# Zeng-Yan/centermask2

Measured on AMD Instinct MI355X. Metric: images/sec whole-node (V2-39-eSE 3x800x1280), higher is better.
Workload: dtype f32; 1 GPU; Full CenterMask2 V-39-eSE (VoVNetV2-FPN + FCOS + CenterROIHeads/SAG-Mask/MaskIoU + ROIAlignV2), bs=8 per GPU, 3x800x1280, end-to-end (BASELINE configs[3]); global_batch=8, per_gpu_batch=8, parallelism=dp1, launch=hip-graph, collective=none, weights=seeded random-init, reference state-dict keys

## Files before the change

### centermask2_amd/csrc/conv.hip

```cpp
#include <algorithm>

#include "conv_args.hpp"

namespace cmk {

__global__ __launch_bounds__(256) void splitk_reduce_kernel(const float* __restrict__ ws, int ksplit, long total_pix, int cout_pad,
                                                           const float* __restrict__ scale, const float* __restrict__ shift, int Cout,
                                                           int relu_upto, const float* __restrict__ res, int res_cs, int res_co,
                                                           float* __restrict__ y, int y_cs, int y_co) {
    const int c4n = cout_pad >> 2;
    const long total = total_pix * c4n;
    for (long i = (long)blockIdx.x * 256 + threadIdx.x; i < total; i += (long)gridDim.x * 256) {
        const long pix = i / c4n;
        const int co = (int)(i - pix * c4n) * 4;
        if (co >= Cout) continue;
        f32x4 s = {0.f, 0.f, 0.f, 0.f};
        for (int z = 0; z < ksplit; ++z) {
            const f32x4 v = *reinterpret_cast<const f32x4*>(ws + ((long)z * total_pix + pix) * cout_pad + co);
            s.x += v.x; s.y += v.y; s.z += v.z; s.w += v.w;
        }
#pragma unroll
        for (int j = 0; j < 4; ++j) {
            const int c = co + j;
            if (c < Cout) {
                float v = s[j] * scale[c] + shift[c];
                if (res) v += res[pix * res_cs + res_co + c];
                if (c < relu_upto) v = fmaxf(v, 0.f);
                y[pix * y_cs + y_co + c] = v;
            }
        }
    }
}

static int validate(const cmk_conv_desc* d) {
    if (!d || !d->x || !d->w || !d->y || !d->scale || !d->shift) return fail(CMK_EINVAL, "conv: null pointer%s", "");
    if (d->ksize != 1 && d->ksize != 3) return fail(CMK_EINVAL, "conv: ksize must be 1 or 3%s", "");
    if (d->stride != 1 && d->stride != 2) return fail(CMK_EINVAL, "conv: stride must be 1 or 2%s", "");
    if (d->ksize == 1 && d->stride != 1) return fail(CMK_EINVAL, "conv: 1x1 stride 2 unsupported%s", "");
    if (d->Cin <= 0 || (d->Cin & 15)) return fail(CMK_EINVAL, "conv: Cin (%s%ld) must be a positive multiple of 16", "", d->Cin);
    if (d->Cout <= 0 || d->N <= 0 || d->H <= 0 || d->W <= 0) return fail(CMK_EINVAL, "conv: empty shape%s", "");
    if ((d->x_cs & 3) || (d->x_co & 3)) return fail(CMK_EINVAL, "conv: input view must be 16-byte aligned per pixel%s", "");
    if (((uintptr_t)d->x & 15) || ((uintptr_t)d->w & 15)) return fail(CMK_EINVAL, "conv: x/w must be 16-byte aligned%s", "");
    if (d->x_co + d->Cin > d->x_cs || d->y_co + d->Cout > d->y_cs) return fail(CMK_EINVAL, "conv: channel view out of range%s", "");
    if (d->res_mode < 0 || d->res_mode > 2 || (d->res_mode && !d->res)) return fail(CMK_EINVAL, "conv: bad residual%s", "");
    if ((d->in_scale == nullptr) != (d->in_shift == nullptr)) return fail(CMK_EINVAL, "conv: in_scale and in_shift come together%s", "");
    if (d->in_scale && d->ksize == 1 && ((long)d->H * d->W) % 256) return fail(CMK_EINVAL, "conv: input affine on a 1x1 conv needs H*W %% 256 == 0%s", "");
    if (d->pool_ws && d->ksize != 1) return fail(CMK_EINVAL, "conv: pooled sums are for 1x1 convs%s", "");
    return CMK_OK;
}

static int validate_multi(const cmk_conv_desc* descs, int n) {
    if (!descs || n < 1 || n > MAXP) return fail(CMK_EINVAL, "conv_multi: need 1..%s%ld problems", "", MAXP);
    bool same_w = true;
    for (int i = 0; i < n; ++i) {
        int rc = validate(&descs[i]);
        if (rc) return rc;
        const cmk_conv_desc *a = &descs[0], *b = &descs[i];
        same_w = same_w && b->w == a->w && b->w_wino == a->w_wino && b->w_wino6 == a->w_wino6 && b->w_split == a->w_split && b->w_splith == a->w_splith;
        if (b->Cin != a->Cin || b->Cout != a->Cout || b->ksize != a->ksize || b->stride != a->stride ||
            b->relu_upto != a->relu_upto || b->in_relu != a->in_relu || b->x_cs != a->x_cs || b->x_co != a->x_co || b->y_cs != a->y_cs ||
            b->y_co != a->y_co || b->res_mode != 0 || b->tune_wm != a->tune_wm || b->tune_sc != a->tune_sc || b->tune_wn != a->tune_wn || (b->in_scale == nullptr) != (a->in_scale == nullptr) ||
            b->gn_ws != a->gn_ws || b->gn_groups != a->gn_groups || b->splitk > 1 || b->pool_ws)
            return fail(CMK_EINVAL, "conv_multi: problems must share channels/views/flags and carry no residual%s", "");
    }
    if ((!same_w || n > 5) && (descs[0].tune_wm != 6 || descs[0].tune_wn != 1) && descs[0].tune_wm != 11)
        return fail(CMK_EINVAL, "conv_multi: different weights per problem / more than 5 problems need tune_wm 6, tune_wn 1 (the F(4x4) map kernels)%s", "");
    for (int i = 0; i < n; ++i)
        if (descs[0].tune_wm == 6 && !descs[i].w_wino6) return fail(CMK_EINVAL, "conv_multi: w_wino6 missing%s", "");
    return CMK_OK;
}

static void fill_problem(ConvProblem& p, const cmk_conv_desc* d) {
    p.x = d->x; p.y = d->y; p.scale = d->scale; p.shift = d->shift;
    p.in_scale = d->in_scale; p.in_shift = d->in_shift;
    p.w = d->w_wino6;
    p.N = d->N; p.H = d->H; p.W = d->W;
    p.Ho = out_size(d->H, d->stride);
    p.Wo = out_size(d->W, d->stride);
    p.tiles_h = p.tiles_w = p.tile_begin = 0;
    p.total_pix = (long)p.N * p.Ho * p.Wo;
}

static int setup_gn(ConvArgs& a, const cmk_conv_desc* d) {
    const int cpg = d->gn_groups > 0 ? d->Cout / d->gn_groups : 0;
    if (d->relu_upto != 0 || d->gn_groups < 1 || d->Cout % d->gn_groups || cpg > 32 || (cpg & (cpg - 1)))
        return fail(CMK_EINVAL, "conv: fused GroupNorm statistics need relu_upto == 0 and a power-of-two group width <= 32%s", "");
    a.gn_ws = d->gn_ws; a.gn_cpg = cpg; a.gn_groups = d->gn_groups;
    return CMK_OK;
}

static int pointwise_mt(const cmk_conv_desc* d, int n) {
    const int cout32 = (d->Cout + 31) / 32;
    const long total_pix = (long)d->N * d->H * d->W;
    if (d->ksize != 1 || n != 1 || cout32 <= 7 || (d->Cin & 31) || d->in_scale || d->in_relu || d->gn_ws || total_pix * d->x_cs * 4 >= (1L << 31))
        return 0;
    if (d->splitk > 1 && (d->tune_wm != 8 || !d->splitk_ws || d->res_mode == 2 || d->pool_ws || (d->Cin >> 4) % (2 * d->splitk))) return 0;
    if (d->res_mode == 2 && ((d->W & 1) || d->pool_ws || (long)d->N * d->Hr * d->Wr * d->res_cs * 4 >= (1L << 31))) return 0;
    if (d->tune_wm == 8) return (d->tune_wn == 4 || d->tune_wn == 2) ? d->tune_wn : 0;
    if (d->tune_wm == 10) return (d->w_split && d->tune_wn == 4 && d->res_mode != 1 && d->splitk <= 1) ? 4 : 0;
    if (d->tune_wm == 12) return (d->w_splith && d->tune_wn == 4 && d->res_mode != 1 && d->splitk <= 1) ? 4 : 0;
    if (d->tune_wm || d->tune_sc || d->tune_wn) return 0;
    const long ctiles = cdiv(cout32, 4);
    const long wg2 = ((total_pix + 127) / 128) * ctiles, wg4 = ((total_pix + 255) / 256) * ctiles;
    return wg2 >= 256 ? (wg4 >= 1024 ? 4 : 2) : 0;
}

static int gather_mt(const cmk_conv_desc* d, int n) {
    const int cout32 = (d->Cout + 31) / 32;
    const long in_pix = (long)d->N * d->H * d->W;
    const long out_pix = (long)d->N * (d->stride == 1 ? d->H : (d->H - 1) / 2 + 1) * (d->stride == 1 ? d->W : (d->W - 1) / 2 + 1);
    if (d->ksize != 3 || n != 1 || (cout32 != 4 && cout32 <= 7) || (d->Cin & 31) || d->in_scale || d->in_relu || d->res_mode == 2 ||
        d->gn_ws || d->pool_ws || in_pix * d->x_cs * 4 >= (1L << 31) || d->H >= 32768 || d->W >= 32768)
        return 0;
    if (d->splitk > 1 && (d->tune_wm != 9 || !d->splitk_ws || (9 * (d->Cin >> 4)) % (2 * d->splitk))) return 0;
    if (d->tune_wm == 9) return (d->tune_wn == 4 || d->tune_wn == 2) ? d->tune_wn : 0;
// ... 105 lines not shown
        if (d->tune_wn != 1 && d->tune_wn != 2) return fail(CMK_EINVAL, "conv: tune_wm 6 takes tune_wn 1 (12x40 map tiles) or 2 (pairs of RoI maps up to 16x14)%s", "");
        if (d->tune_sc == 64) return launch_wino6s(a, d->tune_wn == 2 ? 1 : 0, st, plan);
        return launch_wino6(a, d->tune_wn == 2 ? 1 : 0, pair, st, plan);
    }
    a.ksplit = d->splitk > 1 ? d->splitk : 1;
    a.ws = d->splitk_ws;
    if (d->pool_ws && !pointwise_mt(d, n)) return fail(CMK_EINVAL, "conv: pooled sums are produced by the pointwise GEMM kernel only (cmk_conv_pool_rows)%s", "");
    a.pool_ws = d->pool_ws;
    if (d->tune_wm == 8) {
        if (d->ksize != 1 || cout32 <= 7) return fail(CMK_EINVAL, "conv: pointwise variant needs a 1x1 conv with Cout > 224%s", "");
        a.cout_pad = cout_pad128;
        if (a.ksplit > 1 && !pointwise_mt(d, n)) return fail(CMK_EINVAL, "conv: pointwise variant: split-K not available for this conv%s", "");
        return launch_pw(a, d->tune_wn, st, plan);
    }
    if (d->tune_wm == 10 || d->tune_wm == 12) {
        const bool f16 = d->tune_wm == 12;
        if (!(d->ksize == 1 ? pointwise_mt(d, n) : gather_mt(d, n)) || (f16 && !(d->w_splith_scale > 0.f)))
            return fail(CMK_EINVAL, f16 ? "conv: the fp16-split variant needs w_splith, w_splith_scale and a conv the pointwise GEMM kernel takes (1x1, or 3x3 in its gather form)%s"
                                        : "conv: the bf16-split variant needs w_split and a conv the pointwise GEMM kernel takes (1x1, or 3x3 in its gather form)%s", "");
        a.cout_pad = cout_pad128;
        a.w = reinterpret_cast<const float*>(f16 ? d->w_splith : d->w_split);
        if (f16) a.p[0].acc_scale = d->w_splith_scale;
        a.ksplit = 1;
        a.ga_stride = d->ksize == 3 ? d->stride : 0;
        return launch_pw_split(a, f16 ? 2 : 1, st, plan);
    }
    if (d->tune_wm == 11) {
        if (d->ksize != 3 || d->stride != 1 || !d->w_splith || d->splitk > 1 || d->res_mode != 0 || d->in_relu || d->pool_ws)
            return fail(CMK_EINVAL, "conv: the direct fp16-split variant needs w_splith and a plain 3x3 stride-1 conv%s", "");
        for (int i = 0; i < n; ++i) {
            if (!descs[i].w_splith || !(descs[i].w_splith_scale > 0.f)) return fail(CMK_EINVAL, "conv: w_splith / w_splith_scale missing%s", "");
            a.p[i].w = reinterpret_cast<const float*>(descs[i].w_splith);
            a.p[i].acc_scale = descs[i].w_splith_scale;
        }
        a.cout_pad = cout_pad128;
        a.ksplit = 1;
        return launch_sp3(a, d->tune_wn, d->tune_sc, st, plan);
    }
    if (d->tune_wm == 9) {
        const int mt = gather_mt(d, n);
        if (!mt) return fail(CMK_EINVAL, "conv: pointwise gather variant not available for this conv%s", "");
        a.cout_pad = cout_pad128;
        a.ga_stride = d->stride;
        return launch_pw(a, mt, st, plan);
    }
    if (d->tune_wm == 7) {
        if (d->ksize != 3 || n != 1 || d->res_mode == 2 || d->in_scale || (d->tune_wn != 1 && d->tune_wn != 2 && d->tune_wn != 4))
            return fail(CMK_EINVAL, "conv: gather variant not available for this conv%s", "");
        const int cout_pad32 = cout32 <= 7 ? cout32 : cdiv(cout32, 4) * 4;
        if (cout_pad32 % d->tune_wn) return fail(CMK_EINVAL, "conv: gather variant: Cout tiles %% WN != 0%s", "");
        a.cout_pad = cout_pad32 * 32;
        a.ga_stride = d->stride;
        return launch_igemm_gather(a, d->tune_wn, cout_pad32 / d->tune_wn, st, plan);
    }
    const Variant v{d->tune_wm, d->tune_sc, d->tune_wn};
    if (!variant_ok(d->ksize * d->ksize, d->stride, cout32, v.wm, v.sc, v.wn)) return fail(CMK_EINVAL, "conv: variant not available for this shape%s", "");
    return launch_igemm(a, d->ksize, d->stride, cout32, v, st, plan);
}

static int run(const cmk_conv_desc* descs, int n, void* stream, LaunchPlan* plan = nullptr) {
    const cmk_conv_desc* d = &descs[0];
    ConvArgs a;
    memset(&a, 0, sizeof(a));
    a.nprob = n;
    for (int i = 0; i < n; ++i) fill_problem(a.p[i], &descs[i]);
    a.w = d->w; a.res = d->res;
    a.Cin = d->Cin; a.Cout = d->Cout;
    a.x_cs = d->x_cs; a.x_co = d->x_co; a.y_cs = d->y_cs; a.y_co = d->y_co;
    a.res_cs = d->res_cs; a.res_co = d->res_co; a.res_mode = d->res_mode; a.Hr = d->Hr; a.Wr = d->Wr;
    if (a.res_mode == 2 && (a.Hr * 2 < a.p[0].Ho || a.Wr * 2 < a.p[0].Wo)) return fail(CMK_EINVAL, "conv: upsampled residual too small%s", "");
    a.relu_upto = d->relu_upto; a.in_relu = d->in_relu;
    const bool ask_gn = plan && !d->gn_ws && d->gn_groups > 0;
    const Variant v = resolve(descs, n, d->gn_ws != nullptr || ask_gn);
    cmk_conv_desc dv = *d;
    dv.tune_wm = v.wm; dv.tune_sc = v.sc; dv.tune_wn = v.wn;
    static double no_ws;
    if (ask_gn && writes_gn_records(v.wm)) dv.gn_ws = &no_ws;
    hipStream_t st = (hipStream_t)stream;
    int rc = dispatch(a, &dv, descs, n, st, plan);
    if (rc || plan) return rc;
    if (a.ksplit <= 1 && a.tail_ksplit > 1 && a.tail_tiles > 0) {
        const ConvProblem& p = a.p[0];
        const long pix0 = (long)2 * (a.total_tiles - a.tail_tiles) * p.Ho * p.Wo, tpix = p.total_pix - pix0;
        hipLaunchKernelGGL(splitk_reduce_kernel, dim3((unsigned)std::min<long>((tpix * (a.cout_pad >> 2) + 255) / 256, 256L * 32)), dim3(256), 0, st, a.ws, a.tail_ksplit,
                           tpix, a.cout_pad, p.scale, p.shift, a.Cout, a.relu_upto, (const float*)nullptr, 0, 0, p.y + pix0 * a.y_cs, a.y_cs, a.y_co);
        return check_launch("splitk_reduce (tail)");
    }
    if (a.ksplit <= 1) return rc;
    const ConvProblem& p = a.p[0];
    hipLaunchKernelGGL(splitk_reduce_kernel, dim3((unsigned)std::min<long>((p.total_pix * (a.cout_pad >> 2) + 255) / 256, 256L * 32)), dim3(256), 0, st, a.ws, a.ksplit, p.total_pix,
                       a.cout_pad, p.scale, p.shift, a.Cout, a.relu_upto, a.res_mode == 1 ? a.res : nullptr, a.res_cs, a.res_co, p.y, a.y_cs,
                       a.y_co);
    return check_launch("splitk_reduce");
}

}

extern "C" int cmk_conv_cout_pad(int Cout) {
    int c32 = (Cout + 31) / 32;
    return c32 <= 7 ? c32 * 32 : ((c32 + 3) / 4) * 128;
}

extern "C" int64_t cmk_conv_packed_floats(int Cout, int Cin, int ksize) {
    int64_t taps = (int64_t)ksize * ksize;
    int64_t nch = (Cin + 15) / 16;
    return taps * nch * cmk_conv_cout_pad(Cout) * 16;
}

extern "C" int cmk_conv_gn_tiles(int H, int W) { return ((H + 7) / 8) * ((W + 15) / 16); }

extern "C" int cmk_conv_gn_records(int H, int W, int tune_wm) {
    return tune_wm == 6 ? cmk::wino6_gn_records(H, W) : cmk::wino4r_gn_records(H, W);
}

extern "C" int64_t cmk_splith_packed_halves(int Cout, int Cin) {
    return (int64_t)((Cin + 15) / 16) * (((Cout + 127) / 128) * 4) * 2 * 64 * 8;
}

extern "C" int64_t cmk_split_packed_halves(int Cout, int Cin) {
    return (int64_t)((Cin + 15) / 16) * (((Cout + 127) / 128) * 4) * 3 * 64 * 8;
}

extern "C" int64_t cmk_wino_packed_floats(int Cout, int Cin) {
    return (int64_t)((Cin + 15) / 16) * ((Cout + 63) / 64) * 16 * 64 * 16;
}

extern "C" int cmk_conv_pool_rows(const cmk_conv_desc* d) {
    if (!d) return 0;
    const int mt = cmk::pointwise_mt(d, 1);
    return (mt && (long)d->H * d->W >= 32 * mt) ? 32 * mt : 0;
}

extern "C" int64_t cmk_conv_tail_ws_floats(const cmk_conv_desc* d) {
    if (!d) return 0;
    int tiles = 0, ways = 0;
    cmk::wino6_tail_of(d, tiles, ways);
    if (tiles <= 0 || ways <= 1) return 0;
    const int st = (d->N + 1) / 2;
    const int64_t images = d->N - 2 * (int64_t)(st - tiles);
    return (int64_t)ways * images * d->H * d->W * cmk_conv_cout_pad(d->Cout);
}

extern "C" int cmk_conv2d_nhwc(const cmk_conv_desc* d, void* stream) {
    int rc = cmk::validate(d);
    if (rc) return rc;
    return cmk::run(d, 1, stream);
}

extern "C" int cmk_conv2d_nhwc_multi(const cmk_conv_desc* descs, int n, void* stream) {
    int rc = cmk::validate_multi(descs, n);
    if (rc) return rc;
    return cmk::run(descs, n, stream);
}

extern "C" int cmk_conv_plan(const cmk_conv_desc* descs, int n, char* kernel, int kernel_cap, double* executed_flops, int* gn_records) {
    int rc = n == 1 ? cmk::validate(descs) : cmk::validate_multi(descs, n);
    if (rc) return rc;
    cmk::LaunchPlan plan;
    memset(&plan, 0, sizeof(plan));
    rc = cmk::run(descs, n, nullptr, &plan);
    if (rc) return rc;
    if (kernel && kernel_cap > 0) snprintf(kernel, kernel_cap, "%s", plan.kernel);
    if (executed_flops) *executed_flops = (double)plan.executed_flops;
    for (int i = 0; gn_records && i < n; ++i) gn_records[i] = plan.gn_records[i];
    return CMK_OK;
}

extern "C" int cmk_conv_resolve(const cmk_conv_desc* descs, int n, int with_gn_stats, int variant[3]) {
    int rc = n == 1 ? cmk::validate(descs) : cmk::validate_multi(descs, n);
    if (rc) return rc;
    if (!variant) return cmk::fail(CMK_EINVAL, "conv_resolve: null variant%s", "");
    const cmk::Variant v = cmk::resolve(descs, n, with_gn_stats || descs[0].gn_ws);
    variant[0] = v.wm; variant[1] = v.sc; variant[2] = v.wn;
// ... 3 lines not shown
```

### centermask2_amd/csrc/elementwise.hip

```cpp
#include "cmk_common.hpp"

namespace cmk {

typedef float f32x4 __attribute__((ext_vector_type(4)));
typedef float f32x16 __attribute__((ext_vector_type(16)));

__device__ __forceinline__ float nanmax(float m, float v) { return (v > m || v != v) ? v : m; }
__device__ __forceinline__ float hsigmoid3(float v) {
    v = v < 0.f ? 0.f : v;
    v = v > 6.f ? 6.f : v;
    return v / 6.0f;
}

template <int NB>
__global__ __launch_bounds__(256) void stem_conv_kernel(const float* __restrict__ x, const float* __restrict__ w,
                                                       const float* __restrict__ scale, const float* __restrict__ shift,
                                                       float* __restrict__ y, int N, int H, int W, int Ho, int Wo, long tiles) {
    const int lane = threadIdx.x & 63, wave = threadIdx.x >> 6;
    const int li = lane & 31, hh = lane >> 5;
    constexpr int Cout = NB * 32;
    float b[14][NB], sc[NB], sh[NB];
    int dlt[14], khs[14], kws[14];
#pragma unroll
    for (int s = 0; s < 14; ++s) {
// ... 74 lines not shown

__global__ __launch_bounds__(256) void subsample2_kernel(const float* __restrict__ x, int x_cs, int x_co, float* __restrict__ y, int y_cs, int y_co,
                                                        int N, int H, int W, int Ho, int Wo, int C4) {
    long total = (long)N * Ho * Wo * C4;
    for (long i = (long)blockIdx.x * 256 + threadIdx.x; i < total; i += (long)gridDim.x * 256) {
        int c4 = (int)(i % C4);
        long p = i / C4;
        int ow = (int)(p % Wo);
        int oh = (int)((p / Wo) % Ho);
        int n = (int)(p / ((long)Wo * Ho));
        *reinterpret_cast<f32x4*>(y + p * y_cs + y_co + c4 * 4) =
            *reinterpret_cast<const f32x4*>(x + (((long)n * H + 2 * oh) * W + 2 * ow) * x_cs + x_co + c4 * 4);
    }
}

__global__ __launch_bounds__(256) void ese_partial_kernel(const float* __restrict__ x, int x_cs, int x_co, float* __restrict__ ws,
                                                         int HW, int C, int chunks) {
    extern __shared__ float red[];
    const int n = blockIdx.y, chunk = blockIdx.x;
    const int G = C >> 2;
    const int ppl = G >= 256 ? 1 : 256 / G;
    const int per = cdiv(HW, chunks);
    const int p0 = chunk * per, p1 = min(HW, p0 + per);
    const float* xn = x + (long)n * HW * x_cs + x_co;
    for (int gi = threadIdx.x; gi < G * ppl; gi += 256) {
        int g = gi % G, pl = gi / G;
        f32x4 s = {0.f, 0.f, 0.f, 0.f};
        for (int p = p0 + pl; p < p1; p += ppl) {
            f32x4 v = *reinterpret_cast<const f32x4*>(xn + (long)p * x_cs + g * 4);
            s.x += v.x; s.y += v.y; s.z += v.z; s.w += v.w;
        }
        *reinterpret_cast<f32x4*>(red + pl * C + g * 4) = s;
    }
    __syncthreads();
    for (int c = threadIdx.x; c < C; c += 256) {
        float s = 0.f;
        for (int pl = 0; pl < ppl; ++pl) s += red[pl * C + c];
        ws[((long)n * chunks + chunk) * C + c] = s;
    }
}

__global__ __launch_bounds__(256) void ese_fc_kernel(const float* __restrict__ ws, const float* __restrict__ fc_w,
                                                    const float* __restrict__ fc_b, float* __restrict__ gate, int HW, int C,
                                                    int chunks) {
    extern __shared__ double smd[];
    const int n = blockIdx.y;
    const int G = C >> 2;
    const int parts = G >= 256 ? 1 : 256 / G;
    const float* wsn = ws + (long)n * chunks * C;
    for (int gi = threadIdx.x; gi < G * parts; gi += 256) {
        const int g = gi % G, part = gi / G;
        double s0 = 0.0, s1 = 0.0, s2 = 0.0, s3 = 0.0;
#pragma unroll 8
        for (int k = part; k < chunks; k += parts) {
            const f32x4 v = *reinterpret_cast<const f32x4*>(wsn + (long)k * C + g * 4);
            s0 += (double)v.x; s1 += (double)v.y; s2 += (double)v.z; s3 += (double)v.w;
        }
        double* o = smd + part * C + g * 4;
        o[0] = s0; o[1] = s1; o[2] = s2; o[3] = s3;
    }
    __syncthreads();
    for (int c = threadIdx.x; c < C; c += 256) {
        double s = 0.0;
        for (int part = 0; part < parts; ++part) s += smd[part * C + c];
        smd[c] = s / (double)HW;
    }
    __syncthreads();
    const int lane = threadIdx.x & 63, wave = threadIdx.x >> 6;
    for (int o = blockIdx.x * 16 + wave; o < min(C, (int)(blockIdx.x + 1) * 16); o += 4) {
        const float* wr = fc_w + (long)o * C;
        double s = 0.0;
        for (int c = lane * 4; c < C; c += 256) {
            f32x4 wv = *reinterpret_cast<const f32x4*>(wr + c);
            s += (double)wv.x * smd[c] + (double)wv.y * smd[c + 1] + (double)wv.z * smd[c + 2] + (double)wv.w * smd[c + 3];
        }
        s = wave_sum(s);
        if (lane == 0) {
            float v = (float)(s + (double)fc_b[o] + 3.0);
            gate[(long)n * C + o] = hsigmoid3(v);
        }
    }
}

__global__ __launch_bounds__(256) void ese_fc_pooled_kernel(const float* __restrict__ rec, int rows, const float* __restrict__ fc_w,
                                                           const float* __restrict__ fc_b, float* __restrict__ gate, int HW, int C) {
    extern __shared__ double smd[];
    const int n = blockIdx.y;
    const int G = C >> 2;
    const int parts = G >= 256 ? 1 : 256 / G;
    const long p0 = (long)n * HW;
    const long g0 = p0 / rows, g1 = (p0 + HW - 1) / rows;
    const long first = (g0 * rows == p0) ? 2 * g0 : 2 * g0 + 1;
    for (int gi = threadIdx.x; gi < G * parts; gi += 256) {
        const int g = gi % G, part = gi / G;
        double s0 = 0.0, s1 = 0.0, s2 = 0.0, s3 = 0.0;
        if (part == 0) {
            const f32x4 v = *reinterpret_cast<const f32x4*>(rec + first * C + g * 4);
            s0 = v.x; s1 = v.y; s2 = v.z; s3 = v.w;
        }
#pragma unroll 8
        for (long k = g0 + 1 + part; k <= g1; k += parts) {
            const f32x4 v = *reinterpret_cast<const f32x4*>(rec + 2 * k * C + g * 4);
            s0 += (double)v.x; s1 += (double)v.y; s2 += (double)v.z; s3 += (double)v.w;
        }
        double* o = smd + part * C + g * 4;
        o[0] = s0; o[1] = s1; o[2] = s2; o[3] = s3;
    }
    __syncthreads();
    for (int c = threadIdx.x; c < C; c += 256) {
        double s = 0.0;
        for (int part = 0; part < parts; ++part) s += smd[part * C + c];
        smd[c] = s / (double)HW;
    }
    __syncthreads();
    const int lane = threadIdx.x & 63, wave = threadIdx.x >> 6;
    for (int o = blockIdx.x * 16 + wave; o < min(C, (int)(blockIdx.x + 1) * 16); o += 4) {
        const float* wr = fc_w + (long)o * C;
        double s = 0.0;
        for (int c = lane * 4; c < C; c += 256) {
            f32x4 wv = *reinterpret_cast<const f32x4*>(wr + c);
            s += (double)wv.x * smd[c] + (double)wv.y * smd[c + 1] + (double)wv.z * smd[c + 2] + (double)wv.w * smd[c + 3];
        }
        s = wave_sum(s);
        if (lane == 0) {
            float v = (float)(s + (double)fc_b[o] + 3.0);
            gate[(long)n * C + o] = hsigmoid3(v);
        }
    }
}

__global__ __launch_bounds__(256) void ese_scale_kernel(const float* __restrict__ x, int x_cs, int x_co, const float* __restrict__ gate,
                                                       const float* __restrict__ idn, int id_cs, int id_co, float* __restrict__ y,
                                                       int y_cs, int y_co, int N, int HW, int C4) {
    long total = (long)N * HW * C4;
    for (long i = (long)blockIdx.x * 256 + threadIdx.x; i < total; i += (long)gridDim.x * 256) {
        int c4 = (int)(i % C4);
        long p = i / C4;
        int n = (int)(p / HW);
        f32x4 v = *reinterpret_cast<const f32x4*>(x + p * x_cs + x_co + c4 * 4);
        f32x4 g = *reinterpret_cast<const f32x4*>(gate + (long)n * C4 * 4 + c4 * 4);
        f32x4 o = {v.x * g.x, v.y * g.y, v.z * g.z, v.w * g.w};
        if (idn) {
            f32x4 d = *reinterpret_cast<const f32x4*>(idn + p * id_cs + id_co + c4 * 4);
            o.x += d.x; o.y += d.y; o.z += d.z; o.w += d.w;
        }
        *reinterpret_cast<f32x4*>(y + p * y_cs + y_co + c4 * 4) = o;
    }
}

__global__ __launch_bounds__(256) void upsample2x_add_kernel(float* __restrict__ y, const float* __restrict__ c, int N, int H, int W, int Hc, int Wc, int C4) {
    long total = (long)N * H * W * C4;
    for (long i = (long)blockIdx.x * 256 + threadIdx.x; i < total; i += (long)gridDim.x * 256) {
        int c4 = (int)(i % C4);
        long p = i / C4;
        int w = (int)(p % W);
        int h = (int)((p / W) % H);
        int n = (int)(p / ((long)W * H));
        const f32x4 a = *reinterpret_cast<const f32x4*>(y + i * 4);
        const f32x4 b = *reinterpret_cast<const f32x4*>(c + ((((long)n * Hc + (h >> 1)) * Wc + (w >> 1)) * C4 + c4) * 4);
        *reinterpret_cast<f32x4*>(y + i * 4) = f32x4{a.x + b.x, a.y + b.y, a.z + b.z, a.w + b.w};
    }
}

}

using namespace cmk;

extern "C" int cmk_stem_conv_nchw3(const float* x, const float* w, const float* scale, const float* shift, float* y, int N, int H,
                                   int W, int Cout, void* stream) {
    if (!x || !w || !scale || !shift || !y) return fail(CMK_EINVAL, "stem: null pointer%s", "");
    if (Cout != 32 && Cout != 64 && Cout != 128) return fail(CMK_EINVAL, "stem: Cout (%s%ld) must be 32, 64 or 128", "", (long)Cout);
    int Ho = (H - 1) / 2 + 1, Wo = (W - 1) / 2 + 1;
    long total = (long)N * Ho * Wo;
    if ((long)3 * H * W >= (1L << 31)) return fail(CMK_EINVAL, "stem: image too large%s", "");
    long tiles = (total + 31) / 32;
    unsigned grid = (unsigned)std::min<long>((tiles + 3) / 4, 256 * 16);
    if (Cout == 32)
        hipLaunchKernelGGL(stem_conv_kernel<1>, dim3(grid), dim3(256), 0, (hipStream_t)stream, x, w, scale, shift, y, N, H, W, Ho, Wo, tiles);
    else if (Cout == 64)
        hipLaunchKernelGGL(stem_conv_kernel<2>, dim3(grid), dim3(256), 0, (hipStream_t)stream, x, w, scale, shift, y, N, H, W, Ho, Wo, tiles);
    else
        hipLaunchKernelGGL(stem_conv_kernel<4>, dim3(grid), dim3(256), 0, (hipStream_t)stream, x, w, scale, shift, y, N, H, W, Ho, Wo, tiles);
    return check_launch("stem_conv");
}

extern "C" int cmk_maxpool3x3s2_ceil_nhwc(const float* x, int x_cs, int x_co, float* y, int y_cs, int y_co, int N, int H, int W, int C,
                                          const float* gate, void* stream) {
    if (!x || !y) return fail(CMK_EINVAL, "maxpool: null pointer%s", "");
    if ((C & 3) || (x_cs & 3) || (x_co & 3) || (y_cs & 3) || (y_co & 3)) return fail(CMK_EINVAL, "maxpool: channels must be multiples of 4%s", "");
    if (H < 3 || W < 3) return fail(CMK_EINVAL, "maxpool: input smaller than the window%s", "");
    int Ho = (H - 3 + 1) / 2 + 1, Wo = (W - 3 + 1) / 2 + 1;
    if ((Ho - 1) * 2 >= H) --Ho;
    if ((Wo - 1) * 2 >= W) --Wo;
    long total = (long)N * Ho * Wo * (C >> 2);
    hipLaunchKernelGGL(maxpool3_kernel, dim3(stream_grid(total)), dim3(256), 0, (hipStream_t)stream, x, x_cs, x_co, y, y_cs, y_co, N, H, W,
                       Ho, Wo, C >> 2, gate);
    return check_launch("maxpool3");
}

extern "C" int cmk_maxpool1x1s2_nhwc(const float* x, int x_cs, int x_co, float* y, int y_cs, int y_co, int N, int H, int W, int C, void* stream) {
    if (!x || !y) return fail(CMK_EINVAL, "maxpool1x1s2: null pointer%s", "");
    if ((C & 3) || (x_cs & 3) || (x_co & 3) || (y_cs & 3) || (y_co & 3) || N < 1 || H < 1 || W < 1)
        return fail(CMK_EINVAL, "maxpool1x1s2: channels must be multiples of 4, N, H, W >= 1%s", "");
    const int Ho = (H - 1) / 2 + 1, Wo = (W - 1) / 2 + 1;
    long total = (long)N * Ho * Wo * (C >> 2);
    hipLaunchKernelGGL(subsample2_kernel, dim3(stream_grid(total)), dim3(256), 0, (hipStream_t)stream, x, x_cs, x_co, y, y_cs, y_co, N, H, W, Ho, Wo,
                       C >> 2);
    return check_launch("maxpool1x1s2");
}

extern "C" int cmk_ese_gate(const float* x, int x_cs, int x_co, const float* fc_w, const float* fc_b, float* gate, float* ws,
                            int ws_chunks, int N, int HW, int C, void* stream) {
    if (!x || !fc_w || !fc_b || !gate || !ws) return fail(CMK_EINVAL, "ese_gate: null pointer%s", "");
    if ((C & 3) || (x_cs & 3) || (x_co & 3) || ws_chunks < 1) return fail(CMK_EINVAL, "ese_gate: bad shape%s", "");
    if (N < 1 || HW < 1 || C < 4) return fail(CMK_EINVAL, "ese_gate: N, H*W >= 1 and C >= 4%s", "");
    int G = C >> 2;
    int ppl = G >= 256 ? 1 : 256 / G;
    size_t lds1 = (size_t)ppl * C * sizeof(float);
    hipLaunchKernelGGL(ese_partial_kernel, dim3(ws_chunks, N), dim3(256), lds1, (hipStream_t)stream, x, x_cs, x_co, ws, HW, C, ws_chunks);
    int rc = check_launch("ese_partial");
    if (rc) return rc;
    hipLaunchKernelGGL(ese_fc_kernel, dim3(cdiv(C, 16), N), dim3(256), 2 * lds1 , (hipStream_t)stream, ws, fc_w, fc_b,
                       gate, HW, C, ws_chunks);
    return check_launch("ese_fc");
}

extern "C" int cmk_ese_gate_pooled(const float* pool_ws, int rows, const float* fc_w, const float* fc_b, float* gate, int N, int HW, int C, void* stream) {
    if (!pool_ws || !fc_w || !fc_b || !gate) return fail(CMK_EINVAL, "ese_gate_pooled: null pointer%s", "");
    if ((C & 3) || C < 4 || rows < 1 || HW < rows || N < 1) return fail(CMK_EINVAL, "ese_gate_pooled: bad shape (C %% 4, H*W >= rows)%s", "");
    const int G = C >> 2;
    const int parts = G >= 256 ? 1 : 256 / G;
    hipLaunchKernelGGL(ese_fc_pooled_kernel, dim3(cdiv(C, 16), N), dim3(256), (size_t)parts * C * sizeof(double), (hipStream_t)stream, pool_ws, rows,
                       fc_w, fc_b, gate, HW, C);
    return check_launch("ese_fc_pooled");
}

extern "C" int cmk_ese_scale(const float* x, int x_cs, int x_co, const float* gate, const float* identity, int id_cs, int id_co, float* y,
                             int y_cs, int y_co, int N, int HW, int C, void* stream) {
    if (!x || !gate || !y) return fail(CMK_EINVAL, "ese_scale: null pointer%s", "");
    if ((C & 3) || (x_cs & 3) || (x_co & 3) || (y_cs & 3) || (y_co & 3) || (id_cs & 3) || (id_co & 3))
        return fail(CMK_EINVAL, "ese_scale: channels must be multiples of 4%s", "");
    if (N < 1 || HW < 1) return fail(CMK_EINVAL, "ese_scale: N, H*W >= 1%s", "");
    long total = (long)N * HW * (C >> 2);
    hipLaunchKernelGGL(ese_scale_kernel, dim3(stream_grid(total)), dim3(256), 0, (hipStream_t)stream, x, x_cs, x_co, gate, identity, id_cs,
                       id_co, y, y_cs, y_co, N, HW, C >> 2);
    return check_launch("ese_scale");
}

extern "C" int cmk_upsample2x_add_nhwc(float* y, const float* coarse, int N, int H, int W, int Hc, int Wc, int C, void* stream) {
    if (!y || !coarse) return fail(CMK_EINVAL, "upsample2x_add: null pointer%s", "");
    if ((C & 3) || N < 1 || H < 1 || W < 1 || Hc * 2 < H || Wc * 2 < W) return fail(CMK_EINVAL, "upsample2x_add: C %% 4 == 0 and a coarse map of at least half the size%s", "");
    long total = (long)N * H * W * (C >> 2);
    hipLaunchKernelGGL(upsample2x_add_kernel, dim3(stream_grid(total)), dim3(256), 0, (hipStream_t)stream, y, coarse, N, H, W, Hc, Wc, C >> 2);
    return check_launch("upsample2x_add");
}
```

### centermask2_amd/csrc/roi.hip

```cpp
#include "cmk_common.hpp"

namespace cmk {

typedef float f32x4 __attribute__((ext_vector_type(4)));
constexpr int MAXL = 4;

struct RoiLevels {
    const float* feat[MAXL];
    int H[MAXL], W[MAXL];
    float scale[MAXL];
    int num_levels, min_level;
    int assign_area;
    float canonical_size;
    int canonical_level;
    int aligned;
};

__global__ __launch_bounds__(256) void roi_align_kernel(const RoiLevels L, int C, const float* __restrict__ boxes,
                                                       const int32_t* __restrict__ counts, const float* __restrict__ img_area, int topk,
                                                       int out_size, int sampling_ratio, float* __restrict__ y, int y_cs,
                                                       int32_t* __restrict__ out_level, int num_rois) {
    const int bpr = (out_size * out_size + 3) >> 2;
    const int xq = blockIdx.x >> 3, xcd = blockIdx.x & 7;
    const int r = (xq / bpr) * 8 + xcd;
// ... 33 lines not shown
    const float bin_size_h = roi_height / (float)out_size, bin_size_w = roi_width / (float)out_size;
    const int grid_h = sampling_ratio > 0 ? sampling_ratio : (int)ceilf(roi_height / (float)out_size);
    const int grid_w = sampling_ratio > 0 ? sampling_ratio : (int)ceilf(roi_width / (float)out_size);
    const float count = (float)max(grid_h * grid_w, 1);

    for (int c4 = lane; c4 < C4; c4 += 64) {
        f32x4 acc = {0.f, 0.f, 0.f, 0.f};
        for (int iy = 0; iy < grid_h; ++iy) {
            const float yy = roi_start_h + (float)ph * bin_size_h + ((float)iy + 0.5f) * bin_size_h / (float)grid_h;
            for (int ix = 0; ix < grid_w; ++ix) {
                const float xx = roi_start_w + (float)pw * bin_size_w + ((float)ix + 0.5f) * bin_size_w / (float)grid_w;
                float xq = xx, yq = yy;
                if (yq < -1.0f || yq > (float)height || xq < -1.0f || xq > (float)width) continue;
                if (yq <= 0.f) yq = 0.f;
                if (xq <= 0.f) xq = 0.f;
                int y_low = (int)yq, x_low = (int)xq, y_high, x_high;
                if (y_low >= height - 1) { y_high = y_low = height - 1; yq = (float)y_low; } else y_high = y_low + 1;
                if (x_low >= width - 1) { x_high = x_low = width - 1; xq = (float)x_low; } else x_high = x_low + 1;
                const float ly = yq - (float)y_low, lx = xq - (float)x_low, hy = 1.0f - ly, hx = 1.0f - lx;
                const float w1 = hy * hx, w2 = hy * lx, w3 = ly * hx, w4 = ly * lx;
                const f32x4 v1 = *reinterpret_cast<const f32x4*>(feat + ((long)y_low * width + x_low) * C + c4 * 4);
                const f32x4 v2 = *reinterpret_cast<const f32x4*>(feat + ((long)y_low * width + x_high) * C + c4 * 4);
                const f32x4 v3 = *reinterpret_cast<const f32x4*>(feat + ((long)y_high * width + x_low) * C + c4 * 4);
                const f32x4 v4 = *reinterpret_cast<const f32x4*>(feat + ((long)y_high * width + x_high) * C + c4 * 4);
#pragma unroll
                for (int j = 0; j < 4; ++j) acc[j] += w1 * v1[j] + w2 * v2[j] + w3 * v3[j] + w4 * v4[j];
            }
        }
#pragma unroll
        for (int j = 0; j < 4; ++j) acc[j] /= count;
        *reinterpret_cast<f32x4*>(yo + c4 * 4) = acc;
    }
}

__global__ __launch_bounds__(256) void spatial_attention_kernel(float* __restrict__ x, const float* __restrict__ w,
                                                               const int32_t* __restrict__ counts, int topk, int S, int C) {
    extern __shared__ float sm[];
    const int r = blockIdx.x;
    const int n = r / topk, s = r - n * topk;
    if (s >= counts[n]) return;
    const int P = S * S, C4 = C >> 2;
    float* savg = sm;
    float* smax = sm + P;
    float* satt = sm + 2 * P;
    float* xr = x + (long)r * P * C;
    const int lane = threadIdx.x & 63, wave = threadIdx.x >> 6;
    for (int p = wave; p < P; p += 4) {
        float sum = 0.f, mx = -INFINITY;
        for (int c4 = lane; c4 < C4; c4 += 64) {
            f32x4 v = *reinterpret_cast<const f32x4*>(xr + (long)p * C + c4 * 4);
            sum += (v.x + v.y) + (v.z + v.w);
            mx = fmaxf(mx, fmaxf(fmaxf(v.x, v.y), fmaxf(v.z, v.w)));
        }
        sum = wave_sum(sum);
        mx = wave_max(mx);
        if (lane == 0) { savg[p] = sum / (float)C; smax[p] = mx; }
    }
    __syncthreads();
    for (int p = threadIdx.x; p < P; p += 256) {
        const int h = p / S, ww = p - h * S;
        float a = 0.f;
#pragma unroll
        for (int kh = 0; kh < 3; ++kh)
#pragma unroll
            for (int kw = 0; kw < 3; ++kw) {
                int ih = h + kh - 1, iw = ww + kw - 1;
                if (ih >= 0 && ih < S && iw >= 0 && iw < S) {
                    a += savg[ih * S + iw] * w[kh * 3 + kw];
                    a += smax[ih * S + iw] * w[9 + kh * 3 + kw];
                }
            }
        satt[p] = 1.0f / (1.0f + expf(-a));
    }
    __syncthreads();
    for (int i = threadIdx.x; i < P * C4; i += 256) {
        const int p = i / C4;
        f32x4 v = *reinterpret_cast<f32x4*>(xr + (long)i * 4);
        const float g = satt[p];
        v.x *= g; v.y *= g; v.z *= g; v.w *= g;
        *reinterpret_cast<f32x4*>(xr + (long)i * 4) = v;
    }
}

__global__ __launch_bounds__(256) void mask_predict_kernel(const float* __restrict__ dec, const float* __restrict__ pw,
                                                          const float* __restrict__ pb, const int64_t* __restrict__ cls,
                                                          const int32_t* __restrict__ counts, int topk, int S, int C,
                                                          float* __restrict__ masks, float* __restrict__ logits_opt) {
    const int r = blockIdx.y;
    const int n = r / topk, s = r - n * topk;
    const int lane = threadIdx.x & 63, wave = threadIdx.x >> 6;
    const int q = blockIdx.x * 4 + wave;
    const int P4 = S * S * 4;
    if (q >= P4) return;
    const int sub = q & 3, hw = q >> 2;
    const int h = hw / S, w = hw - h * S;
    const int oh = 2 * h + (sub >> 1), ow = 2 * w + (sub & 1);
    const long o = ((long)r * 2 * S + oh) * 2 * S + ow;
    if (s >= counts[n]) {
        if (lane == 0) { masks[o] = 0.f; if (logits_opt) logits_opt[o] = 0.f; }
        return;
    }
    const int k = (int)cls[r];
    const float* d = dec + ((long)r * P4 + q) * C;
    const float* wv = pw + (long)k * C;
    float acc = 0.f;
    for (int c = lane * 4; c < C; c += 256) {
        f32x4 a = *reinterpret_cast<const f32x4*>(d + c);
        f32x4 b = *reinterpret_cast<const f32x4*>(wv + c);
        acc += a.x * b.x + a.y * b.y + a.z * b.z + a.w * b.w;
    }
    acc = wave_sum(acc);
    if (lane == 0) {
        float lg = acc + pb[k];
        if (logits_opt) logits_opt[o] = lg;
        masks[o] = 1.0f / (1.0f + expf(-lg));
    }
}

__device__ inline float max_nan(float a, float b) { return (a != a || a > b) ? a : b; }

__global__ __launch_bounds__(256) void mask_pool_kernel(const float* __restrict__ masks, float* __restrict__ y, int y_cs, int y_co, int R,
                                                       int S, int pad) {
    long total = (long)R * S * S;
    for (long i = (long)blockIdx.x * 256 + threadIdx.x; i < total; i += (long)gridDim.x * 256) {
        int w = (int)(i % S), h = (int)((i / S) % S);
        long r = i / ((long)S * S);
        const float* m = masks + (r * 2 * S + 2 * h) * 2 * S + 2 * w;
        float v = max_nan(max_nan(m[0], m[1]), max_nan(m[2 * S], m[2 * S + 1]));
        float* o = y + i * y_cs + y_co;
        o[0] = v;
        for (int j = 1; j < pad; ++j) o[j] = 0.f;
    }
}

__global__ void mask_iou_score_kernel(const float* __restrict__ iou, int iou_cs, const float* __restrict__ scores,
                                      const int64_t* __restrict__ cls, float* __restrict__ out, int R) {
    int r = blockIdx.x * blockDim.x + threadIdx.x;
    if (r < R) out[r] = scores[r] * iou[(long)r * iou_cs + cls[r]];
}

}

using namespace cmk;

extern "C" int cmk_roi_align_pool(const float* const* feats, const int* feat_h, const int* feat_w, const float* scales, int num_levels,
                                  int min_level, int C, const float* boxes, const int32_t* counts, const float* img_area, int N,
                                  int topk, int out_size, int sampling_ratio, int aligned, int assign_by_area, float canonical_box_size,
                                  int canonical_level, float* y, int y_cs, int32_t* out_level, void* stream) {
    if (!feats || !feat_h || !feat_w || !scales || !boxes || !counts || (!img_area && !assign_by_area) || !y || !out_level)
        return fail(CMK_EINVAL, "roi_align: null pointer%s", "");
    if (assign_by_area && !(canonical_box_size > 0.f)) return fail(CMK_EINVAL, "roi_align: canonical_box_size must be positive%s", "");
    if (num_levels < 1 || num_levels > MAXL || (C & 3) || y_cs < C || (y_cs & 3) || N < 1 || topk < 1 || out_size < 1)
        return fail(CMK_EINVAL, "roi_align: bad shape%s", "");
    RoiLevels L;
    L.num_levels = num_levels;
    L.min_level = min_level;
    L.assign_area = assign_by_area ? 1 : 0;
    L.canonical_size = canonical_box_size;
    L.canonical_level = canonical_level;
    L.aligned = aligned ? 1 : 0;
    for (int l = 0; l < MAXL; ++l) {
        bool ok = l < num_levels;
        if (ok && !feats[l]) return fail(CMK_EINVAL, "roi_align: null level%s", "");
        L.feat[l] = ok ? feats[l] : nullptr;
        L.H[l] = ok ? feat_h[l] : 1;
        L.W[l] = ok ? feat_w[l] : 1;
        L.scale[l] = ok ? scales[l] : 1.f;
        if (ok && (feat_h[l] < 1 || feat_w[l] < 1)) return fail(CMK_EINVAL, "roi_align: %slevel %ld has no pixels", "", (long)l);
    }
    const long lgrid = (((long)out_size * out_size + 3) / 4) * ((((long)N * topk + 7) / 8) * 8);
    if (lgrid > 0x7fffffffL) return fail(CMK_EINVAL, "roi_align: %s%ld workgroups do not fit the grid", "", lgrid);
    int R = N * topk;
    hipLaunchKernelGGL(roi_align_kernel, dim3(cdiv(out_size * out_size, 4) * (((R + 7) / 8) * 8)), dim3(256), 0, (hipStream_t)stream, L, C, boxes,
                       counts, img_area, topk, out_size, sampling_ratio, y, y_cs, out_level, R);
    return check_launch("roi_align");
}

extern "C" int cmk_roi_align_ratio(const float* const* feats, const int* feat_h, const int* feat_w, const float* scales, int num_levels,
                                   int min_level, int C, const float* boxes, const int32_t* counts, const float* img_area, int N,
                                   int topk, int out_size, int sampling_ratio, float* y, int y_cs, int32_t* out_level, void* stream) {
    return cmk_roi_align_pool(feats, feat_h, feat_w, scales, num_levels, min_level, C, boxes, counts, img_area, N, topk, out_size,
                              sampling_ratio, 1, 0, 224.f, 4, y, y_cs, out_level, stream);
}

extern "C" int cmk_spatial_attention(float* x, const float* w, const int32_t* counts, int topk, int R, int S, int C, void* stream) {
    if (!x || !w || !counts) return fail(CMK_EINVAL, "spatial_attention: null pointer%s", "");
    if ((C & 3) || S < 1 || R < 1 || topk < 1 || R % topk) return fail(CMK_EINVAL, "spatial_attention: bad shape%s", "");
    if (3L * S * S * (long)sizeof(float) > 65536L)
        return fail(CMK_EINVAL, "spatial_attention: %sS = %ld needs %ld bytes of LDS, more than 65536", "", (long)S, 3L * S * S * (long)sizeof(float));
    hipLaunchKernelGGL(spatial_attention_kernel, dim3(R), dim3(256), (size_t)3 * S * S * sizeof(float), (hipStream_t)stream, x, w, counts,
                       topk, S, C);
    return check_launch("spatial_attention");
}

extern "C" int cmk_mask_predict(const float* deconv_out, const float* pw, const float* pb, const int64_t* cls, const int32_t* counts,
                                int topk, int R, int S, int C, float* masks, float* mask_logits_opt, void* stream) {
    if (!deconv_out || !pw || !pb || !cls || !counts || !masks) return fail(CMK_EINVAL, "mask_predict: null pointer%s", "");
    if ((C & 3) || S < 1 || R < 1 || topk < 1 || R % topk) return fail(CMK_EINVAL, "mask_predict: bad shape%s", "");
    if (R > 65535 || (long)S * S > 0x7fffffffL) return fail(CMK_EINVAL, "mask_predict: %s%ld RoIs x %ld pixels do not fit the grid", "", (long)R, (long)S * S);
    hipLaunchKernelGGL(mask_predict_kernel, dim3(S * S, R), dim3(256), 0, (hipStream_t)stream, deconv_out, pw, pb, cls, counts, topk, S, C,
                       masks, mask_logits_opt);
    return check_launch("mask_predict");
}

extern "C" int cmk_mask_pool_concat(const float* masks, float* y, int y_cs, int y_co, int R, int S, void* stream) {
    if (!masks || !y) return fail(CMK_EINVAL, "mask_pool: null pointer%s", "");
    if (R < 1 || S < 1 || y_co < 0 || y_co >= y_cs) return fail(CMK_EINVAL, "mask_pool: bad shape%s", "");
    long total = (long)R * S * S;
    if ((total + 255) / 256 > 0x7fffffffL) return fail(CMK_EINVAL, "mask_pool: %s%ld outputs do not fit the grid", "", total);
    int grid = (int)((total + 255) / 256);
    hipLaunchKernelGGL(mask_pool_kernel, dim3(grid), dim3(256), 0, (hipStream_t)stream, masks, y, y_cs, y_co, R, S, y_cs - y_co);
    return check_launch("mask_pool");
}

extern "C" int cmk_mask_iou_score(const float* iou, int iou_cs, const float* scores, const int64_t* cls, float* mask_scores, int R,
                                  void* stream) {
    if (!iou || !scores || !cls || !mask_scores) return fail(CMK_EINVAL, "mask_iou_score: null pointer%s", "");
    if (R < 1 || iou_cs < 1) return fail(CMK_EINVAL, "mask_iou_score: %sR = %ld RoIs, iou_cs = %ld: need at least 1", "", (long)R, (long)iou_cs);
    hipLaunchKernelGGL(mask_iou_score_kernel, dim3(cdiv(R, 256)), dim3(256), 0, (hipStream_t)stream, iou, iou_cs, scores, cls, mask_scores, R);
    return check_launch("mask_iou_score");
}
```

Baseline: 380.0 images/sec.

## Batch loads in split-K reduce, ESE pooling/FC, and multi-pixel mask predict

The split-K reduce kernel now issues batches of workspace loads before accumulating, writes outputs as 16-byte vectors when aligned, and picks a smaller block size for small problems. The ESE pooled kernel batches its pooling loads and prefetches FC weight rows into registers, with each wave computing several output rows at once. The mask predict kernel has each wave handle four output pixels so the class weight load is shared, and the grid shrinks to match. All of this is meant to raise memory-level parallelism and cut launch granularity. It adds register pressure, and the mask dot product is kept unfused to preserve rounding.

```diff
diff --git a/centermask2_amd/csrc/conv.hip b/centermask2_amd/csrc/conv.hip
--- a/centermask2_amd/csrc/conv.hip
+++ b/centermask2_amd/csrc/conv.hip
@@ -4,21 +4,29 @@
 
 namespace cmk {
 
+constexpr int REDUCE_BATCH = 8;
 __global__ __launch_bounds__(256) void splitk_reduce_kernel(const float* __restrict__ ws, int ksplit, long total_pix, int cout_pad,
                                                            const float* __restrict__ scale, const float* __restrict__ shift, int Cout,
                                                            int relu_upto, const float* __restrict__ res, int res_cs, int res_co,
                                                            float* __restrict__ y, int y_cs, int y_co) {
     const int c4n = cout_pad >> 2;
     const long total = total_pix * c4n;
-    for (long i = (long)blockIdx.x * 256 + threadIdx.x; i < total; i += (long)gridDim.x * 256) {
+    const bool wide = (((y_cs | y_co) & 3) == 0) && (((uintptr_t)y & 15) == 0);
+    for (long i = (long)blockIdx.x * blockDim.x + threadIdx.x; i < total; i += (long)gridDim.x * blockDim.x) {
         const long pix = i / c4n;
         const int co = (int)(i - pix * c4n) * 4;
         if (co >= Cout) continue;
         f32x4 s = {0.f, 0.f, 0.f, 0.f};
-        for (int z = 0; z < ksplit; ++z) {
-            const f32x4 v = *reinterpret_cast<const f32x4*>(ws + ((long)z * total_pix + pix) * cout_pad + co);
-            s.x += v.x; s.y += v.y; s.z += v.z; s.w += v.w;
-        }
+        for (int z0 = 0; z0 < ksplit; z0 += REDUCE_BATCH) {
+            f32x4 v[REDUCE_BATCH];
+#pragma unroll
+            for (int j = 0; j < REDUCE_BATCH; ++j)
+                if (z0 + j < ksplit) v[j] = *reinterpret_cast<const f32x4*>(ws + ((long)(z0 + j) * total_pix + pix) * cout_pad + co);
+#pragma unroll
+            for (int j = 0; j < REDUCE_BATCH; ++j)
+                if (z0 + j < ksplit) { s.x += v[j].x; s.y += v[j].y; s.z += v[j].z; s.w += v[j].w; }
+        }
+        f32x4 o = {0.f, 0.f, 0.f, 0.f};
 #pragma unroll
         for (int j = 0; j < 4; ++j) {
             const int c = co + j;
@@ -26,11 +34,22 @@
                 float v = s[j] * scale[c] + shift[c];
                 if (res) v += res[pix * res_cs + res_co + c];
                 if (c < relu_upto) v = fmaxf(v, 0.f);
-                y[pix * y_cs + y_co + c] = v;
+                o[j] = v;
             }
         }
-    }
-}
+        float* yo = y + pix * y_cs + y_co + co;
+        if (wide && co + 3 < Cout) {
+            *reinterpret_cast<f32x4*>(yo) = o;
+        } else {
+#pragma unroll
+            for (int j = 0; j < 4; ++j)
+                if (co + j < Cout) yo[j] = o[j];
+        }
+    }
+}
+
+static inline unsigned splitk_reduce_block(long quads) { return quads <= 256L * 4 * 256 ? 64u : 256u; }
+static inline unsigned splitk_reduce_grid(long quads, unsigned block) { return (unsigned)std::min<long>(std::max<long>((quads + block - 1) / block, 1L), 256L * 32); }
 
 static int validate(const cmk_conv_desc* d) {
     if (!d || !d->x || !d->w || !d->y || !d->scale || !d->shift) return fail(CMK_EINVAL, "conv: null pointer%s", "");
@@ -302,13 +321,15 @@
     if (a.ksplit <= 1 && a.tail_ksplit > 1 && a.tail_tiles > 0) {
         const ConvProblem& p = a.p[0];
         const long pix0 = (long)2 * (a.total_tiles - a.tail_tiles) * p.Ho * p.Wo, tpix = p.total_pix - pix0;
-        hipLaunchKernelGGL(splitk_reduce_kernel, dim3((unsigned)std::min<long>((tpix * (a.cout_pad >> 2) + 255) / 256, 256L * 32)), dim3(256), 0, st, a.ws, a.tail_ksplit,
+        const unsigned rb = splitk_reduce_block(tpix * (a.cout_pad >> 2));
+        hipLaunchKernelGGL(splitk_reduce_kernel, dim3(splitk_reduce_grid(tpix * (a.cout_pad >> 2), rb)), dim3(rb), 0, st, a.ws, a.tail_ksplit,
                            tpix, a.cout_pad, p.scale, p.shift, a.Cout, a.relu_upto, (const float*)nullptr, 0, 0, p.y + pix0 * a.y_cs, a.y_cs, a.y_co);
         return check_launch("splitk_reduce (tail)");
     }
     if (a.ksplit <= 1) return rc;
     const ConvProblem& p = a.p[0];
-    hipLaunchKernelGGL(splitk_reduce_kernel, dim3((unsigned)std::min<long>((p.total_pix * (a.cout_pad >> 2) + 255) / 256, 256L * 32)), dim3(256), 0, st, a.ws, a.ksplit, p.total_pix,
+    const unsigned rb = splitk_reduce_block(p.total_pix * (a.cout_pad >> 2));
+    hipLaunchKernelGGL(splitk_reduce_kernel, dim3(splitk_reduce_grid(p.total_pix * (a.cout_pad >> 2), rb)), dim3(rb), 0, st, a.ws, a.ksplit, p.total_pix,
                        a.cout_pad, p.scale, p.shift, a.Cout, a.relu_upto, a.res_mode == 1 ? a.res : nullptr, a.res_cs, a.res_co, p.y, a.y_cs,
                        a.y_co);
     return check_launch("splitk_reduce");
diff --git a/centermask2_amd/csrc/elementwise.hip b/centermask2_amd/csrc/elementwise.hip
--- a/centermask2_amd/csrc/elementwise.hip
+++ b/centermask2_amd/csrc/elementwise.hip
@@ -180,12 +180,23 @@
     }
 }
 
+constexpr int ESE_ROWS = 16;
+constexpr int ESE_BATCH = 32;
 __global__ __launch_bounds__(256) void ese_fc_pooled_kernel(const float* __restrict__ rec, int rows, const float* __restrict__ fc_w,
                                                            const float* __restrict__ fc_b, float* __restrict__ gate, int HW, int C) {
     extern __shared__ double smd[];
     const int n = blockIdx.y;
     const int G = C >> 2;
     const int parts = G >= 256 ? 1 : 256 / G;
+    const int lane = threadIdx.x & 63, wave = threadIdx.x >> 6;
+    constexpr int RPW = ESE_ROWS / 4;
+    const int oend = min(C, (int)(blockIdx.x + 1) * ESE_ROWS);
+    f32x4 wn[RPW];
+#pragma unroll
+    for (int j = 0; j < RPW; ++j) {
+        const int o = blockIdx.x * ESE_ROWS + wave + 4 * j;
+        wn[j] = (o < oend && lane * 4 < C) ? *reinterpret_cast<const f32x4*>(fc_w + (long)o * C + lane * 4) : f32x4{0.f, 0.f, 0.f, 0.f};
+    }
     const long p0 = (long)n * HW;
     const long g0 = p0 / rows, g1 = (p0 + HW - 1) / rows;
     const long first = (g0 * rows == p0) ? 2 * g0 : 2 * g0 + 1;
@@ -196,10 +207,14 @@
             const f32x4 v = *reinterpret_cast<const f32x4*>(rec + first * C + g * 4);
             s0 = v.x; s1 = v.y; s2 = v.z; s3 = v.w;
         }
-#pragma unroll 8
-        for (long k = g0 + 1 + part; k <= g1; k += parts) {
-            const f32x4 v = *reinterpret_cast<const f32x4*>(rec + 2 * k * C + g * 4);
-            s0 += (double)v.x; s1 += (double)v.y; s2 += (double)v.z; s3 += (double)v.w;
+        for (long k = g0 + 1 + part; k <= g1; k += (long)ESE_BATCH * parts) {
+            f32x4 v[ESE_BATCH];
+#pragma unroll
+            for (int i = 0; i < ESE_BATCH; ++i)
+                if (k + (long)i * parts <= g1) v[i] = *reinterpret_cast<const f32x4*>(rec + 2 * (k + (long)i * parts) * C + g * 4);
+#pragma unroll
+            for (int i = 0; i < ESE_BATCH; ++i)
+                if (k + (long)i * parts <= g1) { s0 += (double)v[i].x; s1 += (double)v[i].y; s2 += (double)v[i].z; s3 += (double)v[i].w; }
         }
         double* o = smd + part * C + g * 4;
         o[0] = s0; o[1] = s1; o[2] = s2; o[3] = s3;
@@ -211,17 +226,27 @@
         smd[c] = s / (double)HW;
     }
     __syncthreads();
-    const int lane = threadIdx.x & 63, wave = threadIdx.x >> 6;
-    for (int o = blockIdx.x * 16 + wave; o < min(C, (int)(blockIdx.x + 1) * 16); o += 4) {
-        const float* wr = fc_w + (long)o * C;
-        double s = 0.0;
-        for (int c = lane * 4; c < C; c += 256) {
-            f32x4 wv = *reinterpret_cast<const f32x4*>(wr + c);
-            s += (double)wv.x * smd[c] + (double)wv.y * smd[c + 1] + (double)wv.z * smd[c + 2] + (double)wv.w * smd[c + 3];
-        }
-        s = wave_sum(s);
-        if (lane == 0) {
-            float v = (float)(s + (double)fc_b[o] + 3.0);
+    double s[RPW];
+#pragma unroll
+    for (int j = 0; j < RPW; ++j) s[j] = 0.0;
+    for (int c = lane * 4; c < C; c += 256) {
+        f32x4 wv[RPW];
+#pragma unroll
+        for (int j = 0; j < RPW; ++j) {
+            wv[j] = wn[j];
+            const int o = blockIdx.x * ESE_ROWS + wave + 4 * j;
+            if (o < oend && c + 256 < C) wn[j] = *reinterpret_cast<const f32x4*>(fc_w + (long)o * C + c + 256);
+        }
+#pragma unroll
+        for (int j = 0; j < RPW; ++j)
+            s[j] += (double)wv[j].x * smd[c] + (double)wv[j].y * smd[c + 1] + (double)wv[j].z * smd[c + 2] + (double)wv[j].w * smd[c + 3];
+    }
+#pragma unroll
+    for (int j = 0; j < RPW; ++j) {
+        const int o = blockIdx.x * ESE_ROWS + wave + 4 * j;
+        const double t = wave_sum(s[j]);
+        if (lane == 0 && o < oend) {
+            float v = (float)(t + (double)fc_b[o] + 3.0);
             gate[(long)n * C + o] = hsigmoid3(v);
         }
     }
@@ -328,7 +353,7 @@
     if ((C & 3) || C < 4 || rows < 1 || HW < rows || N < 1) return fail(CMK_EINVAL, "ese_gate_pooled: bad shape (C %% 4, H*W >= rows)%s", "");
     const int G = C >> 2;
     const int parts = G >= 256 ? 1 : 256 / G;
-    hipLaunchKernelGGL(ese_fc_pooled_kernel, dim3(cdiv(C, 16), N), dim3(256), (size_t)parts * C * sizeof(double), (hipStream_t)stream, pool_ws, rows,
+    hipLaunchKernelGGL(ese_fc_pooled_kernel, dim3(cdiv(C, ESE_ROWS), N), dim3(256), (size_t)parts * C * sizeof(double), (hipStream_t)stream, pool_ws, rows,
                        fc_w, fc_b, gate, HW, C);
     return check_launch("ese_fc_pooled");
 }
diff --git a/centermask2_amd/csrc/roi.hip b/centermask2_amd/csrc/roi.hip
--- a/centermask2_amd/csrc/roi.hip
+++ b/centermask2_amd/csrc/roi.hip
@@ -139,6 +139,11 @@
     }
 }
 
+constexpr int MP_PPW = 4;
+__device__ __forceinline__ float dot4_unfused(f32x4 a, f32x4 b) {
+#pragma clang fp contract(off)
+    return ((a.x * b.x + a.y * b.y) + a.z * b.z) + a.w * b.w;
+}
 __global__ __launch_bounds__(256) void mask_predict_kernel(const float* __restrict__ dec, const float* __restrict__ pw,
                                                           const float* __restrict__ pb, const int64_t* __restrict__ cls,
                                                           const int32_t* __restrict__ counts, int topk, int S, int C,
@@ -146,29 +151,40 @@
     const int r = blockIdx.y;
     const int n = r / topk, s = r - n * topk;
     const int lane = threadIdx.x & 63, wave = threadIdx.x >> 6;
-    const int q = blockIdx.x * 4 + wave;
+    const int q0 = (blockIdx.x * 4 + wave) * MP_PPW;
     const int P4 = S * S * 4;
-    if (q >= P4) return;
+    if (q0 >= P4) return;
+    const int q = q0 + (lane & (MP_PPW - 1));
     const int sub = q & 3, hw = q >> 2;
     const int h = hw / S, w = hw - h * S;
     const int oh = 2 * h + (sub >> 1), ow = 2 * w + (sub & 1);
     const long o = ((long)r * 2 * S + oh) * 2 * S + ow;
     if (s >= counts[n]) {
-        if (lane == 0) { masks[o] = 0.f; if (logits_opt) logits_opt[o] = 0.f; }
+        if (lane < MP_PPW) { masks[o] = 0.f; if (logits_opt) logits_opt[o] = 0.f; }
         return;
     }
     const int k = (int)cls[r];
-    const float* d = dec + ((long)r * P4 + q) * C;
+    const float* d = dec + ((long)r * P4 + q0) * C;
     const float* wv = pw + (long)k * C;
-    float acc = 0.f;
+    float acc[MP_PPW];
+#pragma unroll
+    for (int j = 0; j < MP_PPW; ++j) acc[j] = 0.f;
     for (int c = lane * 4; c < C; c += 256) {
-        f32x4 a = *reinterpret_cast<const f32x4*>(d + c);
+        f32x4 a[MP_PPW];
+#pragma unroll
+        for (int j = 0; j < MP_PPW; ++j) a[j] = *reinterpret_cast<const f32x4*>(d + (long)j * C + c);
         f32x4 b = *reinterpret_cast<const f32x4*>(wv + c);
-        acc += a.x * b.x + a.y * b.y + a.z * b.z + a.w * b.w;
-    }
-    acc = wave_sum(acc);
-    if (lane == 0) {
-        float lg = acc + pb[k];
+#pragma unroll
+        for (int j = 0; j < MP_PPW; ++j) acc[j] += dot4_unfused(a[j], b);
+    }
+    float mine = 0.f;
+#pragma unroll
+    for (int j = 0; j < MP_PPW; ++j) {
+        const float t = wave_sum(acc[j]);
+        if (lane == j) mine = t;
+    }
+    if (lane < MP_PPW) {
+        float lg = mine + pb[k];
         if (logits_opt) logits_opt[o] = lg;
         masks[o] = 1.0f / (1.0f + expf(-lg));
     }
@@ -255,7 +271,7 @@
     if (!deconv_out || !pw || !pb || !cls || !counts || !masks) return fail(CMK_EINVAL, "mask_predict: null pointer%s", "");
     if ((C & 3) || S < 1 || R < 1 || topk < 1 || R % topk) return fail(CMK_EINVAL, "mask_predict: bad shape%s", "");
     if (R > 65535 || (long)S * S > 0x7fffffffL) return fail(CMK_EINVAL, "mask_predict: %s%ld RoIs x %ld pixels do not fit the grid", "", (long)R, (long)S * S);
-    hipLaunchKernelGGL(mask_predict_kernel, dim3(S * S, R), dim3(256), 0, (hipStream_t)stream, deconv_out, pw, pb, cls, counts, topk, S, C,
+    hipLaunchKernelGGL(mask_predict_kernel, dim3(cdiv(S * S, 4), R), dim3(256), 0, (hipStream_t)stream, deconv_out, pw, pb, cls, counts, topk, S, C,
                        masks, mask_logits_opt);
     return check_launch("mask_predict");
 }
```

Result: no change. 382.1 images/sec (median of 6 runs) (+0.5%).
